# UBC-AWP/vision-sam3-yolo-lameless

Measured on AMD Instinct MI355X. Metric: frames/sec (whole node) for YOLO+SAM3+DINOv3 feature extraction, 1080p clips, higher is better.
Workload: dtype f16; 1 GPU; BASELINE cfg#5, dense schedule: fused per-frame path on a synthetic 5 s @ 30 fps 1080p clip (150 unique BGR frames resident in HBM): YOLOv8-l detect (letterbox 384x640, NMS, scale_boxes; f16 plan) -> SAM (Hiera-B+ image encoder + FPN at 1024x1024, box-prompted mask decoder, 1080p mask + statistics + contour features) + DINOv3 ViT-L/16 embed (224x224) on EVERY frame; per-frame records packed, gathe; parallelism=one clip per GPU, 1 GPU(s), one gather per step, streams=7

## Files before the change

### vision-sam3-yolo-lameless_amd/csrc/common.h

```cpp
#pragma once
#include <hip/hip_runtime.h>
#include <stdint.h>
#include <stdio.h>
#include <stdarg.h>
#include "../../include/lmx.h"

typedef _Float16 half_t;
typedef _Float16 half2_t __attribute__((ext_vector_type(2)));
typedef _Float16 half4_t __attribute__((ext_vector_type(4)));
typedef _Float16 half8_t __attribute__((ext_vector_type(8)));
typedef float f32x4 __attribute__((ext_vector_type(4)));
typedef float f32x16 __attribute__((ext_vector_type(16)));
typedef unsigned int u32x4 __attribute__((ext_vector_type(4)));
typedef unsigned int u32x2 __attribute__((ext_vector_type(2)));

void lmx_set_error(const char* fmt, ...);

#define LMX_REQUIRE(cond, ...)            \
  do {                                    \
    if (!(cond)) {                        \
      lmx_set_error(__VA_ARGS__);         \
      return LMX_EINVAL;                  \
    }                                     \
  } while (0)
// ... 53 lines not shown
  p = p * u + -8.481037793e-09f;
  p = p * u + 2.798429583e-07f;
  p = p * u + -6.151207192e-06f;
  p = p * u + 9.615961466e-05f;
  p = p * u + -1.114801972e-03f;
  p = p * u + 9.814679350e-03f;
  p = p * u + -6.632144717e-02f;
  p = p * u + 3.988863025e-01f;
  const f32x2 g = vc * p;
  return v * g + 0.5f * v;
}
__device__ __forceinline__ float gelu_1(float v) {
  const f32x2 r = gelu_pk(f32x2{v, v});
  return r[0];
}

__device__ __forceinline__ float lmx_act(float v, int act) {
  if (act == LMX_ACT_SILU) return v * __builtin_amdgcn_rcpf(1.0f + __builtin_amdgcn_exp2f(-v * 1.44269504088896340736f));
  if (act == LMX_ACT_GELU) return gelu_1(v);
  if (act == LMX_ACT_RELU) return fmaxf(v, 0.0f);
  return v;
}

typedef __attribute__((address_space(3))) void* lds_ptr_t;

__device__ __forceinline__ void lds_dma16(__amdgpu_buffer_rsrc_t rs, char* dst_lds, unsigned voffset, int soffset) {
  __builtin_amdgcn_raw_ptr_buffer_load_lds(rs, (lds_ptr_t)dst_lds, 16, voffset, soffset, 0, 0);
}

#define LMX_WAIT_CASE(n) \
  if constexpr (N == n) asm volatile("s_waitcnt vmcnt(" #n ")" ::: "memory")
template <int N>
__device__ __forceinline__ void wait_vmcnt() {
  static_assert(N == 0 || N == 1 || N == 2 || N == 3 || N == 4 || N == 6 || N == 8 || N == 9 || N == 12 || N == 16 || N == 18 || N == 24 ||
                    N == 32,
                "add the literal for this count");
  LMX_WAIT_CASE(0);
  LMX_WAIT_CASE(1);
  LMX_WAIT_CASE(2);
  LMX_WAIT_CASE(3);
  LMX_WAIT_CASE(4);
  LMX_WAIT_CASE(6);
  LMX_WAIT_CASE(8);
  LMX_WAIT_CASE(9);
  LMX_WAIT_CASE(12);
  LMX_WAIT_CASE(16);
  LMX_WAIT_CASE(18);
  LMX_WAIT_CASE(24);
  LMX_WAIT_CASE(32);
}
#undef LMX_WAIT_CASE
template <int PT>
__device__ __forceinline__ void wait_tiles(int y) {
  if (y >= 4)
    wait_vmcnt<4 * PT>();
  else if (y == 3)
    wait_vmcnt<3 * PT>();
  else if (y == 2)
    wait_vmcnt<2 * PT>();
  else if (y == 1)
    wait_vmcnt<PT>();
  else
    wait_vmcnt<0>();
}

static inline bool aligned16(const void* p) { return (((uintptr_t)p) & 15) == 0; }

__device__ __forceinline__ float wave_sum(float v) {
#pragma unroll
  for (int o = 32; o > 0; o >>= 1) v += __shfl_xor(v, o, 64);
  return v;
}
__device__ __forceinline__ float wave_max(float v) {
#pragma unroll
  for (int o = 32; o > 0; o >>= 1) v = fmaxf(v, __shfl_xor(v, o, 64));
  return v;
}

__device__ __forceinline__ float act_exact(float v, int act) {
  if (act == LMX_ACT_SILU) return v / (1.0f + expf(-v));
  if (act == LMX_ACT_RELU) return fmaxf(v, 0.0f);
  if (act == LMX_ACT_GELU) return 0.5f * v * (1.0f + erff(v * 0.70710678118654752440f));
// ... 21 lines not shown
```

### vision-sam3-yolo-lameless_amd/csrc/gemm2.hip

```cpp
#include "common.h"
#include <stdlib.h>
#include <type_traits>

#ifdef LMX_DBG_TIMELINE
__device__ unsigned long long lmx_tl[8 * 16384];
extern "C" int lmx_dbg_get_timeline(void* host, int64_t bytes) { return (int)hipMemcpyFromSymbol(host, HIP_SYMBOL(lmx_tl), bytes); }
#define TL(i, v) if (threadIdx.x == 0 && swz < 16384) lmx_tl[swz * 8 + (i)] = (v)
#else
#define TL(i, v)
#endif
namespace lmx_gemm2 {

__device__ __forceinline__ float act_apply(float v, int act) { return lmx_act(v, act); }

constexpr int smem_bytes(int BM, int BN, int BK, int NSTAGE) { return NSTAGE * (BM + BN) * BK * 2 + 2 * BN * 4; }
constexpr int waves_per_simd(int BM, int BN, int BK, int NSTAGE) {
  const int smem = smem_bytes(BM, BN, BK, NSTAGE), nwave = (BM / 64) * (BN / 64);
  const int wps = (smem <= 80 * 1024 ? 2 : 1) * nwave / 4;
  return wps < 1 ? 1 : wps;
}
template <int OUT_DT, int BM, int BN, int BK, int NSTAGE, int AMODE, int STAG, bool GATED = false>
__global__ __launch_bounds__(waves_per_simd(BM, BN, BK, NSTAGE) * 256) void gemm2_kernel(const lmx_gemm_desc p, const int ntiles, const int nt_ok) {
  constexpr int NWAVE = (BM / 64) * (BN / 64);
  constexpr int STAGE_BYTES = (BM + BN) * BK * 2;
  constexpr int A_INSTR = BM * BK * 2 / 1024 / NWAVE;
  constexpr int W_INSTR = BN * BK * 2 / 1024 / NWAVE;
  constexpr int ROWS_PER_INSTR = 1024 / (BK * 2);
  constexpr int CHUNKS = BK / 8;
  constexpr int LA = NSTAGE - 1;
  extern __shared__ __attribute__((aligned(16))) char smem[];
  const int tid = threadIdx.x;
  const int lane = tid & 63;
  const int wave = __builtin_amdgcn_readfirstlane(tid >> 6);
  const int wm = wave % (BM / 64), wn = wave / (BM / 64);

  const int bid = blockIdx.x, xcd = bid & 7;
  const int q = ntiles >> 3, r = ntiles & 7;
  const int base = xcd < r ? xcd * (q + 1) : r * (q + 1) + (xcd - r) * q;
  const int cnt = q + (xcd < r ? 1 : 0);
  const int stride = ((int)gridDim.x + 7 - xcd) >> 3;
  const int NT = (p.N + BN - 1) / BN;
  for (int li = bid >> 3; li < cnt; li += stride) {
  const int swz = base + li;
  const int S_ = p.split_k > 1 ? p.split_k : 1;
  const int tile_ = swz / S_, sp_ = swz - tile_ * S_;
  const int mt = tile_ / NT, nt = tile_ - mt * NT;
  const int m0 = mt * BM, n0 = nt * BN;
  TL(0, (unsigned long long)__builtin_amdgcn_s_getreg((31 << 11) | 4));
  TL(1, (unsigned long long)__builtin_amdgcn_s_getreg((31 << 11) | 20));
  TL(2, wall_clock64());
  TL(5, (unsigned long long)bid);

  const int hw_out = (AMODE == 1) ? p.Ho * p.Wo : 1;
  const int img0 = (AMODE == 1) ? m0 / hw_out : 0;
  const char* Ab = reinterpret_cast<const char*>(p.A) +
                   ((AMODE == 1) ? (int64_t)img0 * p.H * p.W_ * p.lda * 2 : (AMODE == 2 ? (int64_t)0 : (int64_t)m0 * p.lda * 2));
// ... 55 lines not shown
      const int kta = kt - (kt >= nkA ? nkA : 0) - (kt >= 2 * nkA ? nkA : 0);
      const int soff_a = (AMODE == 0) ? kta * (BK * 2) : soff;
#pragma unroll
      for (int j = 0; j < A_INSTR; ++j) {
        char* dst = st + (wave * A_INSTR + j) * 1024;
        lds_dma16(a_rs, dst, kill ? OOB : a_off[j], soff_a);
      }
    } else {
      const int k0 = kt * BK;
      const int tap = k0 / p.Cin, ci0 = k0 - tap * p.Cin;
      const int ky = tap / 3, kx = tap - 3 * ky;
      const int tap_off = ((ky * p.W_ + kx) * (int)p.lda + ci0) * 2;
#pragma unroll
      for (int j = 0; j < A_INSTR; ++j) {
        char* dst = st + (wave * A_INSTR + j) * 1024;
        const int iy = (a_yx[j] >> 16) + ky, ix = (int)(short)(a_yx[j] & 0xffff) + kx;
        const bool ok = (unsigned)iy < (unsigned)p.H && (unsigned)ix < (unsigned)p.W_;
        lds_dma16(a_rs, dst, ok ? a_off[j] + (unsigned)tap_off : OOB, 0);
      }
    }
#pragma unroll
    for (int j = 0; j < W_INSTR; ++j) {
      char* dst = st + BM * BK * 2 + (wave * W_INSTR + j) * 1024;
      lds_dma16(w_rs, dst, kill ? OOB : w_off[j], soff);
    }
  };

  f32x4 acc[4][4];
#pragma unroll
  for (int i = 0; i < 4; ++i)
#pragma unroll
    for (int j = 0; j < 4; ++j) acc[i][j] = f32x4{0.f, 0.f, 0.f, 0.f};

  float* bl = reinterpret_cast<float*>(smem + NSTAGE * STAGE_BYTES);
  float bias_v = 0.f, scale_v = 1.f;
  if (AMODE != 1 && tid < BN && n0 + tid < p.N) {
    if (p.bias && sp_ == 0) bias_v = p.bias[n0 + tid];
    if constexpr (GATED) {
      if (p.scale && tid < BN / 2 && (n0 >> 1) + tid < (p.N >> 1)) scale_v = p.scale[(n0 >> 1) + tid];
    } else {
      if (p.scale) scale_v = p.scale[n0 + tid];
    }
  }

#pragma unroll
  for (int t = 0; t < LA; ++t)
    if (t < nloc) issue(kt0 + t, t);

  const int frow = lane & 15, fq = lane >> 4;
  const int fsw = (BK == 64) ? (frow & 7) : ((-(frow >> 2)) & 3);
  constexpr int PT = A_INSTR + W_INSTR;
  if constexpr (STAG == 0) {
  for (int kt = 0; kt < nloc; ++kt) {
    const int left = nloc - 1 - kt;
    wait_tiles<PT>(left < LA - 1 ? left : LA - 1);
    __builtin_amdgcn_s_barrier();
#ifdef LMX_DBG_TIMELINE
    if (kt == 0) { TL(6, wall_clock64()); }
    if (kt == 1) { TL(7, wall_clock64()); }
#endif
    if (kt + LA < nloc) issue(kt0 + kt + LA, (kt + LA) % NSTAGE);
    const char* st = smem + (kt % NSTAGE) * STAGE_BYTES;
    const half_t* as = reinterpret_cast<const half_t*>(st) + (wm * 64 + frow) * BK;
    const half_t* ws = reinterpret_cast<const half_t*>(st + BM * BK * 2) + (wn * 64 + frow) * BK;
#ifdef LMX_DBG_NOMFMA
    if (p.M < 0)
#endif
// ... 30 lines not shown
#pragma unroll
    for (int ks = 0; ks < BK / 32; ++ks) {
      const int coff = (((ks << 2) + fq) ^ fsw) << 3;
#pragma unroll
      for (int j = 0; j < 4; ++j) wf[ks][j] = *reinterpret_cast<const half8_t*>(ws + j * 16 * BK + coff);
#pragma unroll
      for (int i = 0; i < 4; ++i) af[ks][i] = *reinterpret_cast<const half8_t*>(as + i * 16 * BK + coff);
    }
    if (kt + 1 < nloc) {
      const int rest = nloc - 2 - kt;
      wait_tiles<PT>(rest < LA - 2 ? (rest < 0 ? 0 : rest) : (LA - 2 < 0 ? 0 : LA - 2));
    }
    if (kt + LA < nloc) issue(kt0 + kt + LA, (kt + LA) % NSTAGE);
    asm volatile("s_waitcnt lgkmcnt(0)" ::: "memory");
    __builtin_amdgcn_s_barrier();
    __builtin_amdgcn_s_setprio(1);
#pragma unroll
    for (int ks = 0; ks < BK / 32; ++ks)
#pragma unroll
      for (int i = 0; i < 4; ++i)
#pragma unroll
        for (int j = 0; j < 4; ++j)
          acc[i][j] = __builtin_amdgcn_mfma_f32_16x16x32_f16(wf[ks][j], af[ks][i], acc[i][j], 0, 0, 0);
    __builtin_amdgcn_s_setprio(0);
    __builtin_amdgcn_s_barrier();
  }
  if (!grp) __builtin_amdgcn_s_barrier();
  }

  if (AMODE == 1 && tid < BN && n0 + tid < p.N) {
    if (p.bias && sp_ == 0) bias_v = p.bias[n0 + tid];
    if (p.scale) scale_v = p.scale[n0 + tid];
  }
  if (tid < BN) {
    bl[tid] = bias_v;
    bl[BN + tid] = scale_v;
  }
  asm volatile("s_waitcnt lgkmcnt(0)" ::: "memory");
  __builtin_amdgcn_s_barrier();
  TL(3, wall_clock64());
#ifdef LMX_DBG_NOEPI
  if (p.M > 0 && acc[0][0][0] != 12345.f) continue;
#endif
  const bool nt_out = nt_ok && OUT_DT == LMX_F16 && ((p.ldc * 2) & 127) == 0 && (int64_t)p.M * p.N >= (16ll << 20);
  char* my = smem + wave * 4608;
  auto epilogue = [&](auto act_c, auto scale_c) {
    constexpr int ACT = decltype(act_c)::value;
    constexpr bool SCALE = decltype(scale_c)::value;
    const float* blj = bl + wn * 64 + fq * 4;
    auto finish = [&](f32x4 v, int j) -> f32x4 {
      v += *reinterpret_cast<const f32x4*>(blj + j * 16);
      if constexpr (ACT == LMX_ACT_GELU) {
        const f32x2 g0 = gelu_pk(f32x2{v[0], v[1]}), g1 = gelu_pk(f32x2{v[2], v[3]});
        v = f32x4{g0[0], g0[1], g1[0], g1[1]};
      } else if constexpr (ACT != LMX_ACT_NONE) {
#pragma unroll
        for (int e = 0; e < 4; ++e) v[e] = act_apply(v[e], ACT);
      }
      if constexpr (SCALE) v *= *reinterpret_cast<const f32x4*>(blj + BN + j * 16);
      return v;
    };
    if constexpr (ACT == LMX_ACT_SWIGLU) {
      if constexpr (OUT_DT == LMX_F16 && AMODE == 0) {
        half_t* t16 = reinterpret_cast<half_t*>(my);
        constexpr int RS = 40;
        const bool nt_g = nt_ok && ((p.ldc * 2) & 127) == 0 && (int64_t)p.M * p.N >= (32ll << 20);
// ... 132 lines not shown
          const int m = m0 + wm * 64 + pass * 16 + row;
          if (m < p.M && n < p.N) {
            if (has_res) o += rr[it];
            *reinterpret_cast<f32x4*>(Cs + (int64_t)m * p.ldc + n) = o;
          }
        }
      }
    }
  };
  {
    using T = std::true_type;
    using F = std::false_type;
    const int act = p.act;
    if constexpr (GATED) {
      if (p.scale) epilogue(std::integral_constant<int, LMX_ACT_SWIGLU>{}, T{});
      else epilogue(std::integral_constant<int, LMX_ACT_SWIGLU>{}, F{});
    } else if (p.scale) {
      if (act == LMX_ACT_NONE) epilogue(std::integral_constant<int, LMX_ACT_NONE>{}, T{});
      else if (act == LMX_ACT_SILU) epilogue(std::integral_constant<int, LMX_ACT_SILU>{}, T{});
      else if (act == LMX_ACT_GELU) epilogue(std::integral_constant<int, LMX_ACT_GELU>{}, T{});
      else epilogue(std::integral_constant<int, LMX_ACT_RELU>{}, T{});
    } else {
      if (act == LMX_ACT_NONE) epilogue(std::integral_constant<int, LMX_ACT_NONE>{}, F{});
      else if (act == LMX_ACT_SILU) epilogue(std::integral_constant<int, LMX_ACT_SILU>{}, F{});
      else if (act == LMX_ACT_GELU) epilogue(std::integral_constant<int, LMX_ACT_GELU>{}, F{});
      else epilogue(std::integral_constant<int, LMX_ACT_RELU>{}, F{});
    }
  }
  __builtin_amdgcn_s_barrier();
  TL(4, wall_clock64());
  }
}

template <int BM, int BN, int BK, int NSTAGE, int AMODE, int STAG = 0>
int launch2(const lmx_gemm_desc& d, hipStream_t st) {
  const int MT = (d.M + BM - 1) / BM, NT = (d.N + BN - 1) / BN;
  const size_t smem = smem_bytes(BM, BN, BK, NSTAGE);
  int dev;
  LMX_TRY(lmx_stream_device(st, &dev));
  LMX_TRY(lmx_allow_lds(reinterpret_cast<const void*>(&gemm2_kernel<LMX_F16, BM, BN, BK, NSTAGE, AMODE, STAG>), (int)smem, dev));
  LMX_TRY(lmx_allow_lds(reinterpret_cast<const void*>(&gemm2_kernel<LMX_F32, BM, BN, BK, NSTAGE, AMODE, STAG>), (int)smem, dev));
  const int ntiles = MT * NT * (d.split_k > 1 ? d.split_k : 1);
  int grid = ntiles;
  static const int persist = lmx_env_int("LMX_GEMM2_PERSIST", 0);
  static const int nt_ok = !lmx_env_set("LMX_GEMM2_NO_NT");
  if (persist > 0 && grid > 256 * persist) grid = 256 * persist;
  if (d.act == LMX_ACT_SWIGLU) {
    if constexpr (AMODE == 0) {
      LMX_TRY(lmx_allow_lds(reinterpret_cast<const void*>(&gemm2_kernel<LMX_F16, BM, BN, BK, NSTAGE, AMODE, STAG, true>), (int)smem, dev));
      hipLaunchKernelGGL((gemm2_kernel<LMX_F16, BM, BN, BK, NSTAGE, AMODE, STAG, true>), dim3(grid), dim3(BM * BN / 64), smem, st, d, ntiles, nt_ok);
      return lmx_launch_check("gemm2_kernel (gated)");
    } else {
      return LMX_EINVAL;
    }
  }
  if (d.out_dtype == LMX_F16)
    hipLaunchKernelGGL((gemm2_kernel<LMX_F16, BM, BN, BK, NSTAGE, AMODE, STAG>), dim3(grid), dim3(BM * BN / 64), smem, st, d, ntiles, nt_ok);
  else
    hipLaunchKernelGGL((gemm2_kernel<LMX_F32, BM, BN, BK, NSTAGE, AMODE, STAG>), dim3(grid), dim3(BM * BN / 64), smem, st, d, ntiles, nt_ok);
  return lmx_launch_check("gemm2_kernel");
}

constexpr int RL_BM = 128, RL_BN = 448, RL_BK = 64, RL_NSTAGE = 2;
constexpr int RL_STAGE_BYTES = (RL_BM + RL_BN) * RL_BK * 2;
constexpr int RL_RS = RL_BN + 4;
constexpr int RL_SMEM = RL_NSTAGE * RL_STAGE_BYTES + 3 * RL_BN * 4;
static_assert(2 * 32 * RL_RS * 4 <= RL_NSTAGE * RL_STAGE_BYTES, "two 32-row epilogue buffers inside the ring");

__device__ __forceinline__ void wave_sum4(float (&v)[4]) {
#pragma unroll
  for (int o = 32; o > 0; o >>= 1) {
    float t[4];
#pragma unroll
    for (int r = 0; r < 4; ++r) t[r] = __shfl_xor(v[r], o, 64);
#pragma unroll
    for (int r = 0; r < 4; ++r) v[r] += t[r];
  }
}

__global__ __launch_bounds__(512) void gemm2_rowln_kernel(const lmx_gemm_desc p) {
  constexpr int BM = RL_BM, BN = RL_BN, BK = RL_BK, NSTAGE = RL_NSTAGE, STAGE_BYTES = RL_STAGE_BYTES;
  constexpr int NWAVE = 8;
  constexpr int A_INSTR = BM * BK * 2 / 1024 / NWAVE;
  constexpr int W_INSTR = BN * BK * 2 / 1024 / NWAVE;
  constexpr int FJ = BN / 4 / 16;
  extern __shared__ __attribute__((aligned(16))) char smem[];
  const int tid = threadIdx.x;
  const int lane = tid & 63;
  const int wave = __builtin_amdgcn_readfirstlane(tid >> 6);
  const int wm = wave & 1, wn = wave >> 1;
  const int swz = blockIdx.x;
  const int m0 = swz * BM;
// ... 151 lines not shown
          *reinterpret_cast<half4_t*>(Lh + (int64_t)m * p.ld_ln + c0) = half4_t{(half_t)o[0], (half_t)o[1], (half_t)o[2], (half_t)o[3]};
        }
        if (ok1) {
          const f32x4 o = (v1[rr] - mean[rr]) * rstd[rr] * g1 + b1;
          *reinterpret_cast<half4_t*>(Lh + (int64_t)m * p.ld_ln + c1) = half4_t{(half_t)o[0], (half_t)o[1], (half_t)o[2], (half_t)o[3]};
        }
      }
    }
  }
  TL(4, wall_clock64());
}

int launch_rowln(const lmx_gemm_desc& d, hipStream_t st) {
  int dev;
  LMX_TRY(lmx_stream_device(st, &dev));
  LMX_TRY(lmx_allow_lds(reinterpret_cast<const void*>(&gemm2_rowln_kernel), RL_SMEM, dev));
  hipLaunchKernelGGL(gemm2_rowln_kernel, dim3((d.M + RL_BM - 1) / RL_BM), dim3(512), RL_SMEM, st, d);
  return lmx_launch_check("gemm2_rowln_kernel");
}

}
using namespace lmx_gemm2;

static int g_variant = -1;
extern "C" void lmx_dbg_set_gemm2_variant(int v) { g_variant = v; }

static constexpr GemmRoute tiling(int BM, int BN, int BK, int NSTAGE, int STAG = 0) { return GemmRoute{true, BM, BN, BK, NSTAGE, STAG}; }

GemmRoute lmx_gemm2_tiling(const lmx_gemm_desc& d) {
  if (g_variant < 0) g_variant = lmx_env_char("LMX_GEMM2_VARIANT");
  if (d.a_mode == 2) return tiling(256, 256, 64, 2);
  if (d.a_mode == 1) {
    static const int conv_small = lmx_env_set("LMX_GEMM2_CONV_SMALL");
    const int64_t t256 = (int64_t)((d.M + 255) / 256) * ((d.N + 255) / 256);
    const double q256 = (double)t256 / (double)(((t256 + 255) / 256) * 256);
    if (!conv_small && d.N % 256 == 0 && t256 >= 230 && q256 >= 0.75) return tiling(256, 256, 32, 3, 1);
    return tiling(256, 128, 32, 3);
  }
  switch (g_variant) {
    case 'A': return tiling(256, 128, 64, 3);
    case 'B': return tiling(128, 128, 64, 2);
    case 'C': return tiling(256, 128, 32, 3);
    case 'D': return tiling(256, 128, 32, 2);
    case 'E': return tiling(256, 256, 32, 3);
    case 'F': return tiling(256, 256, 32, 4);
    case 'H': return tiling(128, 128, 32, 2);
    case 'I': return tiling(128, 128, 32, 3);
    case 'S': return tiling(256, 128, 32, 6, 1);
    case 'T': return tiling(256, 128, 64, 3, 1);
    case 'U': return tiling(256, 128, 32, 3, 1);
    case 'V': return tiling(256, 128, 32, 4, 1);
    case 'W': return tiling(256, 256, 32, 4, 1);
    case 'Y': return tiling(256, 256, 32, 3, 1);
    case 'Z': return tiling(256, 256, 64, 2);
  }
  const int64_t nt256 = (d.N + 255) / 256, tiles256 = (int64_t)((d.M + 255) / 256) * nt256;
  const double nfrac = (double)d.N / (double)(nt256 * 256);
  const double q256 = (double)tiles256 / (double)(((tiles256 + 255) / 256) * 256);
  if (d.K >= 448 && tiles256 >= 200 && q256 >= 0.75 && nfrac >= 0.85) {
    return tiling(256, 256, 64, 2);
  }
  if (d.K < 448 && d.N >= 224 && d.N <= 1536 && d.N % 256 != 0 && nfrac >= 0.85 && tiles256 >= 200 && q256 >= 0.75)
    return d.K > 128 ? tiling(256, 256, 32, 3) : tiling(256, 256, 64, 2);
  const int64_t tiles = (int64_t)((d.M + 255) / 256) * ((d.N + 127) / 128);
  return (d.K >= 1792 || tiles <= 256) ? tiling(256, 128, 64, 3, 1) : tiling(256, 128, 32, 3);
}

static constexpr int64_t tiling_key(int BM, int BN, int BK, int NSTAGE, int a_mode, int STAG) {
  return ((((int64_t)BM * 1024 + BN) * 1024 + BK) * 16 + NSTAGE) * 16 + a_mode * 2 + STAG;
}

int lmx_gemm2_launch(const lmx_gemm_desc& d, const GemmRoute& r, hipStream_t st) {
  if (r.rowln) return launch_rowln(d, st);
#define LMX_T(BM, BN, BK, NSTAGE, AMODE, STAG) \
  case tiling_key(BM, BN, BK, NSTAGE, AMODE, STAG): return launch2<BM, BN, BK, NSTAGE, AMODE, STAG>(d, st)
  switch (tiling_key(r.BM, r.BN, r.BK, r.NSTAGE, d.a_mode, r.STAG)) {
    LMX_T(256, 256, 64, 2, 2, 0);
    LMX_T(256, 256, 32, 3, 1, 1);
    LMX_T(256, 128, 32, 3, 1, 0);
    LMX_T(256, 128, 64, 3, 0, 0);
    LMX_T(128, 128, 64, 2, 0, 0);
    LMX_T(256, 128, 32, 3, 0, 0);
    LMX_T(256, 128, 32, 2, 0, 0);
    LMX_T(256, 256, 32, 3, 0, 0);
    LMX_T(256, 256, 32, 4, 0, 0);
    LMX_T(128, 128, 32, 2, 0, 0);
    LMX_T(128, 128, 32, 3, 0, 0);
    LMX_T(256, 128, 32, 6, 0, 1);
    LMX_T(256, 128, 64, 3, 0, 1);
    LMX_T(256, 128, 32, 3, 0, 1);
    LMX_T(256, 128, 32, 4, 0, 1);
    LMX_T(256, 256, 32, 4, 0, 1);
    LMX_T(256, 256, 32, 3, 0, 1);
    LMX_T(256, 256, 64, 2, 0, 0);
  }
#undef LMX_T
  LMX_REQUIRE(false, "lmx_k_gemm: no LDS-DMA kernel %dx%dx%d, %d slots, staggered %d for a_mode %d", r.BM, r.BN, r.BK, r.NSTAGE, r.STAG, d.a_mode);
}
```

### vision-sam3-yolo-lameless_amd/csrc/yolo.hip

```cpp
#include "common.h"

namespace {

inline int grid_for(int64_t total, int block = 256) {
  int64_t g = (total + block - 1) / block;
  if (g > 256 * 8) g = 256 * 8;
  if (g < 1) g = 1;
  return (int)g;
}

__global__ __launch_bounds__(256) void letterbox_kernel(const uint8_t* __restrict__ src, uint8_t* __restrict__ dst, int n,
                                                        int sh, int sw, int rh, int rw, int top, int left, int oh, int ow,
                                                        const int* __restrict__ xofs, const short* __restrict__ ialpha,
                                                        const int* __restrict__ yofs, const short* __restrict__ ibeta,
                                                        int swap_rb, int identity) {
  const int64_t total = (int64_t)n * oh * ow;
  for (int64_t i = (int64_t)blockIdx.x * blockDim.x + threadIdx.x; i < total; i += (int64_t)gridDim.x * blockDim.x) {
    const int ox = (int)(i % ow);
    const int64_t r = i / ow;
    const int oy = (int)(r % oh);
    const int img = (int)(r / oh);
    uint8_t* d = dst + i * 3;
    const int dy = oy - top, dx = ox - left;
    if (dy < 0 || dy >= rh || dx < 0 || dx >= rw) {
// ... 7 lines not shown
      v[0] = s[0];
      v[1] = s[1];
      v[2] = s[2];
    } else {
      const int sx0 = xofs[dx];
      const int sx1 = sx0 + 1 < sw ? sx0 + 1 : sw - 1;
      const int a0 = ialpha[2 * dx], a1 = ialpha[2 * dx + 1];
      int sy0 = yofs[dy], sy1 = yofs[dy] + 1;
      sy0 = sy0 < 0 ? 0 : (sy0 < sh ? sy0 : sh - 1);
      sy1 = sy1 < 0 ? 0 : (sy1 < sh ? sy1 : sh - 1);
      const int b0 = ibeta[2 * dy], b1 = ibeta[2 * dy + 1];
      const uint8_t* r0 = S + (int64_t)sy0 * sw * 3;
      const uint8_t* r1 = S + (int64_t)sy1 * sw * 3;
#pragma unroll
      for (int c = 0; c < 3; ++c) {
        const int h0 = (int)r0[sx0 * 3 + c] * a0 + (int)r0[sx1 * 3 + c] * a1;
        const int h1 = (int)r1[sx0 * 3 + c] * a0 + (int)r1[sx1 * 3 + c] * a1;
        const int val = (((b0 * (h0 >> 4)) >> 16) + ((b1 * (h1 >> 4)) >> 16) + 2) >> 2;
        v[c] = (uint8_t)(val < 0 ? 0 : (val > 255 ? 255 : val));
      }
    }
    if (swap_rb) {
      d[0] = v[2];
      d[1] = v[1];
      d[2] = v[0];
    } else {
      d[0] = v[0];
      d[1] = v[1];
      d[2] = v[2];
    }
  }
}

template <int CO_T>
__global__ __launch_bounds__(256) void stem_conv_kernel(const uint8_t* __restrict__ img, const float* __restrict__ w,
                                                        const float* __restrict__ bias, half_t* __restrict__ out, int n,
                                                        int H, int W, int Ho, int Wo, int Cout) {
  extern __shared__ __attribute__((aligned(16))) char smem[];
  float* ws = reinterpret_cast<float*>(smem);
  for (int i = threadIdx.x; i < 27 * Cout; i += blockDim.x) ws[i] = w[i];
  for (int i = threadIdx.x; i < Cout; i += blockDim.x) ws[27 * Cout + i] = bias[i];
  __syncthreads();
  const int64_t total = (int64_t)n * Ho * Wo;
  for (int64_t i = (int64_t)blockIdx.x * blockDim.x + threadIdx.x; i < total; i += (int64_t)gridDim.x * blockDim.x) {
    const int ox = (int)(i % Wo);
    const int64_t r = i / Wo;
    const int oy = (int)(r % Ho);
    const int b = (int)(r / Ho);
    float x[27];
#pragma unroll
    for (int ky = 0; ky < 3; ++ky)
#pragma unroll
      for (int kx = 0; kx < 3; ++kx) {
        const int iy = oy * 2 - 1 + ky, ix = ox * 2 - 1 + kx;
        const bool ok = (unsigned)iy < (unsigned)H && (unsigned)ix < (unsigned)W;
        const uint8_t* s = img + (((int64_t)b * H + (ok ? iy : 0)) * W + (ok ? ix : 0)) * 3;
#pragma unroll
        for (int c = 0; c < 3; ++c) x[(ky * 3 + kx) * 3 + c] = ok ? (float)s[c] / 255.0f : 0.0f;
      }
    half_t* o = out + i * Cout;
    for (int c0 = 0; c0 < Cout; c0 += CO_T) {
      float acc[CO_T];
#pragma unroll
      for (int j = 0; j < CO_T; ++j) acc[j] = ws[27 * Cout + c0 + j];
#pragma unroll
      for (int t = 0; t < 27; ++t) {
        const float xv = x[t];
#pragma unroll
        for (int j = 0; j < CO_T; ++j) acc[j] = fmaf(xv, ws[t * Cout + c0 + j], acc[j]);
      }
      half8_t hv;
#pragma unroll
      for (int j = 0; j < CO_T; ++j) {
        const float v = acc[j] / (1.0f + expf(-acc[j]));
        hv[j] = (half_t)v;
      }
      *reinterpret_cast<half8_t*>(o + c0) = hv;
    }
  }
}

__global__ __launch_bounds__(256) void maxpool5_kernel(const half_t* __restrict__ src, int64_t lds, half_t* __restrict__ dst,
                                                       int64_t ldd, int n, int H, int W, int C) {
  const int cc = C / 8;
  const int64_t total = (int64_t)n * H * W * cc;
  for (int64_t i = (int64_t)blockIdx.x * blockDim.x + threadIdx.x; i < total; i += (int64_t)gridDim.x * blockDim.x) {
    const int c = (int)(i % cc) * 8;
    const int64_t p = i / cc;
    const int x = (int)(p % W);
    const int64_t r = p / W;
    const int y = (int)(r % H);
    const int b = (int)(r / H);
    half8_t m;
#pragma unroll
    for (int e = 0; e < 8; ++e) m[e] = (half_t)(-65504.0f);
    for (int dy = -2; dy <= 2; ++dy) {
      const int yy = y + dy;
      if ((unsigned)yy >= (unsigned)H) continue;
      for (int dx = -2; dx <= 2; ++dx) {
        const int xx = x + dx;
        if ((unsigned)xx >= (unsigned)W) continue;
        const half8_t v = *reinterpret_cast<const half8_t*>(src + (((int64_t)b * H + yy) * W + xx) * lds + c);
#pragma unroll
        for (int e = 0; e < 8; ++e) m[e] = v[e] > m[e] ? v[e] : m[e];
      }
    }
    *reinterpret_cast<half8_t*>(dst + p * ldd + c) = m;
  }
}

__global__ __launch_bounds__(256) void upsample2_kernel(const half_t* __restrict__ src, int64_t lds, half_t* __restrict__ dst,
// ... 142 lines not shown
  for (int l = 0; l < 3; ++l) {
    LMX_REQUIRE(hw[2 * l] > 0 && hw[2 * l + 1] > 0, "lmx_k_pose_gather: level %d geometry", l);
    L.h[l] = hw[2 * l];
    L.w[l] = hw[2 * l + 1];
    L.off[l] = off;
    L.stride[l] = strides[l];
    off += L.h[l] * L.w[l];
  }
  hipLaunchKernelGGL(pose_gather_kernel, dim3(grid_for((int64_t)n * max_det * K)), dim3(256), 0,
                     reinterpret_cast<hipStream_t>(stream), L, ldk, src, counts, n, max_det, K, ndim, padx, pady, gain, w, h, out);
  return lmx_launch_check("pose_gather_kernel");
}

extern "C" int lmx_k_letterbox(const uint8_t* src, uint8_t* dst, int n, int sh, int sw, int rh, int rw, int top, int left,
                               int oh, int ow, const int32_t* xofs, const int16_t* ialpha, const int32_t* yofs,
                               const int16_t* ibeta, int swap_rb, lmx_stream_t stream) {
  LMX_REQUIRE(src && dst, "lmx_k_letterbox: null pointer");
  LMX_REQUIRE(n > 0 && sh > 0 && sw > 0 && rh > 0 && rw > 0 && oh >= top + rh && ow >= left + rw && top >= 0 && left >= 0,
              "lmx_k_letterbox: geometry");
  const int identity = (rh == sh && rw == sw) ? 1 : 0;
  LMX_REQUIRE(identity || (xofs && ialpha && yofs && ibeta), "lmx_k_letterbox: null tables");
  hipLaunchKernelGGL(letterbox_kernel, dim3(grid_for((int64_t)n * oh * ow)), dim3(256), 0,
                     reinterpret_cast<hipStream_t>(stream), src, dst, n, sh, sw, rh, rw, top, left, oh, ow, xofs, ialpha, yofs,
                     ibeta, swap_rb, identity);
  return lmx_launch_check("letterbox_kernel");
}

extern "C" int lmx_k_stem_conv(const uint8_t* img, const float* w, const float* bias, void* out, int n, int H, int W, int Cout,
                               lmx_stream_t stream) {
  LMX_REQUIRE(img && w && bias && out, "lmx_k_stem_conv: null pointer");
  LMX_REQUIRE(n > 0 && H > 0 && W > 0 && Cout > 0 && Cout % 8 == 0 && Cout <= 256, "lmx_k_stem_conv: shape (Cout %d)", Cout);
  LMX_REQUIRE(aligned16(out), "lmx_k_stem_conv: out alignment");
  const int Ho = (H + 2 - 3) / 2 + 1, Wo = (W + 2 - 3) / 2 + 1;
  const size_t smem = (size_t)28 * Cout * sizeof(float);
  hipLaunchKernelGGL((stem_conv_kernel<8>), dim3(grid_for((int64_t)n * Ho * Wo)), dim3(256), smem,
                     reinterpret_cast<hipStream_t>(stream), img, w, bias, reinterpret_cast<half_t*>(out), n, H, W, Ho, Wo, Cout);
  return lmx_launch_check("stem_conv_kernel");
}

extern "C" int lmx_k_maxpool5(const void* src, int64_t lds, void* dst, int64_t ldd, int n, int H, int W, int C,
                              lmx_stream_t stream) {
  LMX_REQUIRE(src && dst, "lmx_k_maxpool5: null pointer");
  LMX_REQUIRE(n > 0 && H > 0 && W > 0 && C > 0 && C % 8 == 0 && lds % 8 == 0 && ldd % 8 == 0 && lds >= C && ldd >= C,
              "lmx_k_maxpool5: shape");
  LMX_REQUIRE(aligned16(src) && aligned16(dst), "lmx_k_maxpool5: alignment");
  hipLaunchKernelGGL(maxpool5_kernel, dim3(grid_for((int64_t)n * H * W * (C / 8))), dim3(256), 0,
                     reinterpret_cast<hipStream_t>(stream), reinterpret_cast<const half_t*>(src), lds,
                     reinterpret_cast<half_t*>(dst), ldd, n, H, W, C);
  return lmx_launch_check("maxpool5_kernel");
}

extern "C" int lmx_k_upsample2(const void* src, int64_t lds, void* dst, int64_t ldd, int n, int H, int W, int C,
                               lmx_stream_t stream) {
  LMX_REQUIRE(src && dst, "lmx_k_upsample2: null pointer");
  LMX_REQUIRE(n > 0 && H > 0 && W > 0 && C > 0 && C % 8 == 0 && lds % 8 == 0 && ldd % 8 == 0 && lds >= C && ldd >= C,
              "lmx_k_upsample2: shape");
  LMX_REQUIRE(aligned16(src) && aligned16(dst), "lmx_k_upsample2: alignment");
  hipLaunchKernelGGL(upsample2_kernel, dim3(grid_for((int64_t)n * 4 * H * W * (C / 8))), dim3(256), 0,
                     reinterpret_cast<hipStream_t>(stream), reinterpret_cast<const half_t*>(src), lds,
                     reinterpret_cast<half_t*>(dst), ldd, n, H, W, C);
  return lmx_launch_check("upsample2_kernel");
}

extern "C" int lmx_k_detect_decode(const float* head, int64_t ldh, float* pred, int n, int H, int W, int nc, float stride,
                                   int a_off, int A, lmx_stream_t stream) {
  LMX_REQUIRE(head && pred, "lmx_k_detect_decode: null pointer");
  LMX_REQUIRE(n > 0 && H > 0 && W > 0 && nc > 0 && a_off >= 0 && a_off + H * W <= A, "lmx_k_detect_decode: shape");
  LMX_REQUIRE(ldh >= 64 + nc && ldh % 4 == 0 && aligned16(head), "lmx_k_detect_decode: head row stride %lld", (long long)ldh);
  hipLaunchKernelGGL(detect_decode_kernel, dim3(grid_for((int64_t)n * H * W * 4)), dim3(256), 0,
// ... 12 lines not shown
```

Measured before the change: 802.0 frames/s.

## Rewrite YOLO stem conv with register weights and add deeper conv GEMM tilings

The YOLO stem conv is restructured so that each thread keeps the weights for a group of 4 output channels in registers. The input patches are staged through double-buffered LDS using a u8-to-float lookup table, and the next chunk's gather is prefetched while the current one is computed. Two new f16-only implicit-GEMM conv tilings (256x256x64 and 256x64x64, 2 stages) are selected for large-K or 64-channel convolutions. Those tilings place the bias/scale scratch inside the ring so occupancy stays at two waves per SIMD. This adds an extra barrier, more vmcnt literals and register pressure in the stem.

```diff
diff --git a/vision-sam3-yolo-lameless_amd/csrc/common.h b/vision-sam3-yolo-lameless_amd/csrc/common.h
--- a/vision-sam3-yolo-lameless_amd/csrc/common.h
+++ b/vision-sam3-yolo-lameless_amd/csrc/common.h
@@ -109,8 +109,8 @@
   if constexpr (N == n) asm volatile("s_waitcnt vmcnt(" #n ")" ::: "memory")
 template <int N>
 __device__ __forceinline__ void wait_vmcnt() {
-  static_assert(N == 0 || N == 1 || N == 2 || N == 3 || N == 4 || N == 6 || N == 8 || N == 9 || N == 12 || N == 16 || N == 18 || N == 24 ||
-                    N == 32,
+  static_assert(N == 0 || N == 1 || N == 2 || N == 3 || N == 4 || N == 6 || N == 8 || N == 9 || N == 10 || N == 12 ||
+                    N == 16 || N == 18 || N == 20 || N == 24 || N == 30 || N == 32 || N == 40,
                 "add the literal for this count");
   LMX_WAIT_CASE(0);
   LMX_WAIT_CASE(1);
@@ -120,11 +120,15 @@
   LMX_WAIT_CASE(6);
   LMX_WAIT_CASE(8);
   LMX_WAIT_CASE(9);
+  LMX_WAIT_CASE(10);
   LMX_WAIT_CASE(12);
   LMX_WAIT_CASE(16);
   LMX_WAIT_CASE(18);
+  LMX_WAIT_CASE(20);
   LMX_WAIT_CASE(24);
+  LMX_WAIT_CASE(30);
   LMX_WAIT_CASE(32);
+  LMX_WAIT_CASE(40);
 }
 #undef LMX_WAIT_CASE
 template <int PT>
diff --git a/vision-sam3-yolo-lameless_amd/csrc/gemm2.hip b/vision-sam3-yolo-lameless_amd/csrc/gemm2.hip
--- a/vision-sam3-yolo-lameless_amd/csrc/gemm2.hip
+++ b/vision-sam3-yolo-lameless_amd/csrc/gemm2.hip
@@ -13,15 +13,24 @@
 
 __device__ __forceinline__ float act_apply(float v, int act) { return lmx_act(v, act); }
 
-constexpr int smem_bytes(int BM, int BN, int BK, int NSTAGE) { return NSTAGE * (BM + BN) * BK * 2 + 2 * BN * 4; }
-constexpr int waves_per_simd(int BM, int BN, int BK, int NSTAGE) {
-  const int smem = smem_bytes(BM, BN, BK, NSTAGE), nwave = (BM / 64) * (BN / 64);
+constexpr bool bl_in_ring(int BM, int BN, int BK, int NSTAGE, int AMODE) {
+  const int ring = NSTAGE * (BM + BN) * BK * 2;
+  return AMODE == 1 && ring <= 80 * 1024 && ring + 2 * BN * 4 > 80 * 1024;
+}
+constexpr int smem_bytes(int BM, int BN, int BK, int NSTAGE, int AMODE = 0) {
+  return NSTAGE * (BM + BN) * BK * 2 + (bl_in_ring(BM, BN, BK, NSTAGE, AMODE) ? 0 : 2 * BN * 4);
+}
+constexpr int waves_per_simd(int BM, int BN, int BK, int NSTAGE, int AMODE = 0) {
+  const int smem = smem_bytes(BM, BN, BK, NSTAGE, AMODE), nwave = (BM / 64) * (BN / 64);
   const int wps = (smem <= 80 * 1024 ? 2 : 1) * nwave / 4;
   return wps < 1 ? 1 : wps;
 }
 template <int OUT_DT, int BM, int BN, int BK, int NSTAGE, int AMODE, int STAG, bool GATED = false>
-__global__ __launch_bounds__(waves_per_simd(BM, BN, BK, NSTAGE) * 256) void gemm2_kernel(const lmx_gemm_desc p, const int ntiles, const int nt_ok) {
+__global__ __launch_bounds__(waves_per_simd(BM, BN, BK, NSTAGE, AMODE) * 256) void gemm2_kernel(const lmx_gemm_desc p, const int ntiles, const int nt_ok) {
   constexpr int NWAVE = (BM / 64) * (BN / 64);
+  constexpr bool BL_IN_RING = bl_in_ring(BM, BN, BK, NSTAGE, AMODE);
+  static_assert(BM * BK * 2 / 1024 >= NWAVE && BN * BK * 2 / 1024 >= NWAVE, "every wave issues at least one LDS-DMA of A and of W per k-tile");
+  static_assert(NWAVE * 4608 <= NSTAGE * (BM + BN) * BK * 2 - (BL_IN_RING ? 2 * BN * 4 : 0), "the epilogue's per-wave slices lie inside the ring");
   constexpr int STAGE_BYTES = (BM + BN) * BK * 2;
   constexpr int A_INSTR = BM * BK * 2 / 1024 / NWAVE;
   constexpr int W_INSTR = BN * BK * 2 / 1024 / NWAVE;
@@ -143,7 +152,7 @@
 #pragma unroll
     for (int j = 0; j < 4; ++j) acc[i][j] = f32x4{0.f, 0.f, 0.f, 0.f};
 
-  float* bl = reinterpret_cast<float*>(smem + NSTAGE * STAGE_BYTES);
+  float* bl = reinterpret_cast<float*>(smem + NSTAGE * STAGE_BYTES - (BL_IN_RING ? 2 * BN * 4 : 0));
   float bias_v = 0.f, scale_v = 1.f;
   if (AMODE != 1 && tid < BN && n0 + tid < p.N) {
     if (p.bias && sp_ == 0) bias_v = p.bias[n0 + tid];
@@ -240,6 +249,10 @@
     if (p.bias && sp_ == 0) bias_v = p.bias[n0 + tid];
     if (p.scale) scale_v = p.scale[n0 + tid];
   }
+  if constexpr (BL_IN_RING) {
+    asm volatile("s_waitcnt lgkmcnt(0)" ::: "memory");
+    __builtin_amdgcn_s_barrier();
+  }
   if (tid < BN) {
     bl[tid] = bias_v;
     bl[BN + tid] = scale_v;
@@ -438,14 +451,15 @@
   }
 }
 
-template <int BM, int BN, int BK, int NSTAGE, int AMODE, int STAG = 0>
+template <int BM, int BN, int BK, int NSTAGE, int AMODE, int STAG = 0, bool F32_TOO = true>
 int launch2(const lmx_gemm_desc& d, hipStream_t st) {
   const int MT = (d.M + BM - 1) / BM, NT = (d.N + BN - 1) / BN;
-  const size_t smem = smem_bytes(BM, BN, BK, NSTAGE);
+  const size_t smem = smem_bytes(BM, BN, BK, NSTAGE, AMODE);
   int dev;
   LMX_TRY(lmx_stream_device(st, &dev));
   LMX_TRY(lmx_allow_lds(reinterpret_cast<const void*>(&gemm2_kernel<LMX_F16, BM, BN, BK, NSTAGE, AMODE, STAG>), (int)smem, dev));
-  LMX_TRY(lmx_allow_lds(reinterpret_cast<const void*>(&gemm2_kernel<LMX_F32, BM, BN, BK, NSTAGE, AMODE, STAG>), (int)smem, dev));
+  if constexpr (F32_TOO)
+    LMX_TRY(lmx_allow_lds(reinterpret_cast<const void*>(&gemm2_kernel<LMX_F32, BM, BN, BK, NSTAGE, AMODE, STAG>), (int)smem, dev));
   const int ntiles = MT * NT * (d.split_k > 1 ? d.split_k : 1);
   int grid = ntiles;
   static const int persist = lmx_env_int("LMX_GEMM2_PERSIST", 0);
@@ -460,10 +474,14 @@
       return LMX_EINVAL;
     }
   }
-  if (d.out_dtype == LMX_F16)
+  if (d.out_dtype == LMX_F16) {
     hipLaunchKernelGGL((gemm2_kernel<LMX_F16, BM, BN, BK, NSTAGE, AMODE, STAG>), dim3(grid), dim3(BM * BN / 64), smem, st, d, ntiles, nt_ok);
-  else
-    hipLaunchKernelGGL((gemm2_kernel<LMX_F32, BM, BN, BK, NSTAGE, AMODE, STAG>), dim3(grid), dim3(BM * BN / 64), smem, st, d, ntiles, nt_ok);
+  } else {
+    if constexpr (F32_TOO)
+      hipLaunchKernelGGL((gemm2_kernel<LMX_F32, BM, BN, BK, NSTAGE, AMODE, STAG>), dim3(grid), dim3(BM * BN / 64), smem, st, d, ntiles, nt_ok);
+    else
+      LMX_REQUIRE(false, "lmx_k_gemm: the %dx%dx%d tiling is built for f16 output only", BM, BN, BK);
+  }
   return lmx_launch_check("gemm2_kernel");
 }
 
@@ -681,9 +699,12 @@
   if (d.a_mode == 2) return tiling(256, 256, 64, 2);
   if (d.a_mode == 1) {
     static const int conv_small = lmx_env_set("LMX_GEMM2_CONV_SMALL");
+    const bool deep = d.out_dtype == LMX_F16 && d.split_k <= 1 && d.Cin % 64 == 0;
     const int64_t t256 = (int64_t)((d.M + 255) / 256) * ((d.N + 255) / 256);
     const double q256 = (double)t256 / (double)(((t256 + 255) / 256) * 256);
-    if (!conv_small && d.N % 256 == 0 && t256 >= 230 && q256 >= 0.75) return tiling(256, 256, 32, 3, 1);
+    if (!conv_small && d.N % 256 == 0 && t256 >= 230 && q256 >= 0.75)
+      return deep && d.K >= 2304 ? tiling(256, 256, 64, 2) : tiling(256, 256, 32, 3, 1);
+    if (deep && d.N == 64 && d.Cin == 64 && d.M >= 65536) return tiling(256, 64, 64, 2);
     return tiling(256, 128, 32, 3);
   }
   switch (g_variant) {
@@ -723,10 +744,14 @@
   if (r.rowln) return launch_rowln(d, st);
 #define LMX_T(BM, BN, BK, NSTAGE, AMODE, STAG) \
   case tiling_key(BM, BN, BK, NSTAGE, AMODE, STAG): return launch2<BM, BN, BK, NSTAGE, AMODE, STAG>(d, st)
+#define LMX_T16(BM, BN, BK, NSTAGE, AMODE, STAG) \
+  case tiling_key(BM, BN, BK, NSTAGE, AMODE, STAG): return launch2<BM, BN, BK, NSTAGE, AMODE, STAG, false>(d, st)
   switch (tiling_key(r.BM, r.BN, r.BK, r.NSTAGE, d.a_mode, r.STAG)) {
     LMX_T(256, 256, 64, 2, 2, 0);
     LMX_T(256, 256, 32, 3, 1, 1);
     LMX_T(256, 128, 32, 3, 1, 0);
+    LMX_T16(256, 64, 64, 2, 1, 0);
+    LMX_T16(256, 256, 64, 2, 1, 0);
     LMX_T(256, 128, 64, 3, 0, 0);
     LMX_T(128, 128, 64, 2, 0, 0);
     LMX_T(256, 128, 32, 3, 0, 0);
@@ -744,5 +769,6 @@
     LMX_T(256, 256, 64, 2, 0, 0);
   }
 #undef LMX_T
+#undef LMX_T16
   LMX_REQUIRE(false, "lmx_k_gemm: no LDS-DMA kernel %dx%dx%d, %d slots, staggered %d for a_mode %d", r.BM, r.BN, r.BK, r.NSTAGE, r.STAG, d.a_mode);
 }
diff --git a/vision-sam3-yolo-lameless_amd/csrc/yolo.hip b/vision-sam3-yolo-lameless_amd/csrc/yolo.hip
--- a/vision-sam3-yolo-lameless_amd/csrc/yolo.hip
+++ b/vision-sam3-yolo-lameless_amd/csrc/yolo.hip
@@ -63,51 +63,108 @@
   }
 }
 
-template <int CO_T>
+constexpr int STEM_CO = 4;
+constexpr int STEM_XS = 28;
+inline int stem_pixb(int Cout) { return 256 / (Cout / STEM_CO); }
+inline int stem_passes(int Cout) { const int pb = stem_pixb(Cout); return pb >= 128 ? 1 : 128 / pb; }
 __global__ __launch_bounds__(256) void stem_conv_kernel(const uint8_t* __restrict__ img, const float* __restrict__ w,
                                                         const float* __restrict__ bias, half_t* __restrict__ out, int n,
-                                                        int H, int W, int Ho, int Wo, int Cout) {
+                                                        int H, int W, int Ho, int Wo, int Cout, int PIXB, int passes, int64_t nchunks) {
   extern __shared__ __attribute__((aligned(16))) char smem[];
-  float* ws = reinterpret_cast<float*>(smem);
-  for (int i = threadIdx.x; i < 27 * Cout; i += blockDim.x) ws[i] = w[i];
-  for (int i = threadIdx.x; i < Cout; i += blockDim.x) ws[27 * Cout + i] = bias[i];
+  float* lut = reinterpret_cast<float*>(smem);
+  float* xs = lut + 256;
+  const int tid = threadIdx.x;
+  const int G = Cout / STEM_CO, CP = PIXB * passes;
+  const bool worker = tid < PIXB * G;
+  const int g = tid % G, lp0 = tid / G;
+  const int64_t total = (int64_t)n * Ho * Wo;
+  lut[tid] = (float)tid / 255.0f;
+
+  f32x2 wr[27][STEM_CO / 2], br[STEM_CO / 2];
+#pragma unroll
+  for (int h = 0; h < STEM_CO / 2; ++h) br[h] = f32x2{bias[g * STEM_CO + 2 * h], bias[g * STEM_CO + 2 * h + 1]};
+#pragma unroll
+  for (int t = 0; t < 27; ++t)
+#pragma unroll
+    for (int h = 0; h < STEM_CO / 2; ++h) wr[t][h] = f32x2{w[t * Cout + g * STEM_CO + 2 * h], w[t * Cout + g * STEM_CO + 2 * h + 1]};
+
+  int v[27];
+  unsigned inside = 0;
+  auto request = [&](int64_t P0) {
+    const int64_t gp = P0 + tid;
+    if (tid < CP && gp < total) {
+      const int ox = (int)(gp % Wo);
+      const int64_t r = gp / Wo;
+      const int oy = (int)(r % Ho);
+      const int64_t b = r / Ho;
+      inside = 0;
+#pragma unroll
+      for (int ky = 0; ky < 3; ++ky)
+#pragma unroll
+        for (int kx = 0; kx < 3; ++kx) {
+          const int iy = oy * 2 - 1 + ky, ix = ox * 2 - 1 + kx;
+          const bool ok = (unsigned)iy < (unsigned)H && (unsigned)ix < (unsigned)W;
+          const uint8_t* s = img + ((b * H + (ok ? iy : 0)) * W + (ok ? ix : 0)) * 3;
+          inside |= (ok ? 1u : 0u) << (ky * 3 + kx);
+#pragma unroll
+          for (int c = 0; c < 3; ++c) v[(ky * 3 + kx) * 3 + c] = s[c];
+        }
+    }
+  };
+  auto stage = [&](int64_t P0, float* dst) {
+    if (tid < CP && P0 + tid < total) {
+      float* d = dst + tid * STEM_XS;
+#pragma unroll
+      for (int t = 0; t < 27; ++t) {
+        const float f = lut[v[t]];
+        d[t] = ((inside >> (t / 3)) & 1) ? f : 0.0f;
+      }
+      d[27] = 0.0f;
+    }
+  };
+
+  int64_t c = blockIdx.x;
+  request(c * CP);
   __syncthreads();
-  const int64_t total = (int64_t)n * Ho * Wo;
-  for (int64_t i = (int64_t)blockIdx.x * blockDim.x + threadIdx.x; i < total; i += (int64_t)gridDim.x * blockDim.x) {
-    const int ox = (int)(i % Wo);
-    const int64_t r = i / Wo;
-    const int oy = (int)(r % Ho);
-    const int b = (int)(r / Ho);
-    float x[27];
-#pragma unroll
-    for (int ky = 0; ky < 3; ++ky)
-#pragma unroll
-      for (int kx = 0; kx < 3; ++kx) {
-        const int iy = oy * 2 - 1 + ky, ix = ox * 2 - 1 + kx;
-        const bool ok = (unsigned)iy < (unsigned)H && (unsigned)ix < (unsigned)W;
-        const uint8_t* s = img + (((int64_t)b * H + (ok ? iy : 0)) * W + (ok ? ix : 0)) * 3;
-#pragma unroll
-        for (int c = 0; c < 3; ++c) x[(ky * 3 + kx) * 3 + c] = ok ? (float)s[c] / 255.0f : 0.0f;
-      }
-    half_t* o = out + i * Cout;
-    for (int c0 = 0; c0 < Cout; c0 += CO_T) {
-      float acc[CO_T];
-#pragma unroll
-      for (int j = 0; j < CO_T; ++j) acc[j] = ws[27 * Cout + c0 + j];
-#pragma unroll
-      for (int t = 0; t < 27; ++t) {
-        const float xv = x[t];
-#pragma unroll
-        for (int j = 0; j < CO_T; ++j) acc[j] = fmaf(xv, ws[t * Cout + c0 + j], acc[j]);
-      }
-      half8_t hv;
-#pragma unroll
-      for (int j = 0; j < CO_T; ++j) {
-        const float v = acc[j] / (1.0f + expf(-acc[j]));
-        hv[j] = (half_t)v;
-      }
-      *reinterpret_cast<half8_t*>(o + c0) = hv;
-    }
+  stage(c * CP, xs);
+  __syncthreads();
+  for (int it = 0; c < nchunks; c += gridDim.x, ++it) {
+    const int64_t P0 = c * CP, Pn = (c + gridDim.x) * CP;
+    const float* cur = xs + (it & 1) * CP * STEM_XS;
+    if (c + gridDim.x < nchunks) request(Pn);
+    if (worker) {
+      for (int ps = 0; ps < passes; ++ps) {
+        const int lp = lp0 + ps * PIXB;
+        const int64_t gp = P0 + lp;
+        if (gp >= total) break;
+        float x[STEM_XS];
+#pragma unroll
+        for (int q = 0; q < STEM_XS / 4; ++q) {
+          const f32x4 xv = *reinterpret_cast<const f32x4*>(cur + lp * STEM_XS + q * 4);
+          x[q * 4 + 0] = xv[0];
+          x[q * 4 + 1] = xv[1];
+          x[q * 4 + 2] = xv[2];
+          x[q * 4 + 3] = xv[3];
+        }
+        f32x2 acc[STEM_CO / 2];
+#pragma unroll
+        for (int h = 0; h < STEM_CO / 2; ++h) acc[h] = br[h];
+#pragma unroll
+        for (int t = 0; t < 27; ++t)
+#pragma unroll
+          for (int h = 0; h < STEM_CO / 2; ++h) acc[h] = __builtin_elementwise_fma(f32x2{x[t], x[t]}, wr[t][h], acc[h]);
+        half4_t hv;
+#pragma unroll
+        for (int j = 0; j < STEM_CO; ++j) {
+          const float a = acc[j >> 1][j & 1];
+          const float s = a / (1.0f + expf(-a));
+          hv[j] = (half_t)s;
+        }
+        *reinterpret_cast<half4_t*>(out + gp * Cout + g * STEM_CO) = hv;
+      }
+    }
+    if (c + gridDim.x < nchunks) stage(Pn, xs + ((it + 1) & 1) * CP * STEM_XS);
+    __syncthreads();
   }
 }
 
@@ -316,9 +373,11 @@
   LMX_REQUIRE(n > 0 && H > 0 && W > 0 && Cout > 0 && Cout % 8 == 0 && Cout <= 256, "lmx_k_stem_conv: shape (Cout %d)", Cout);
   LMX_REQUIRE(aligned16(out), "lmx_k_stem_conv: out alignment");
   const int Ho = (H + 2 - 3) / 2 + 1, Wo = (W + 2 - 3) / 2 + 1;
-  const size_t smem = (size_t)28 * Cout * sizeof(float);
-  hipLaunchKernelGGL((stem_conv_kernel<8>), dim3(grid_for((int64_t)n * Ho * Wo)), dim3(256), smem,
-                     reinterpret_cast<hipStream_t>(stream), img, w, bias, reinterpret_cast<half_t*>(out), n, H, W, Ho, Wo, Cout);
+  const int PIXB = stem_pixb(Cout), passes = stem_passes(Cout), CP = PIXB * passes;
+  const int64_t nchunks = ((int64_t)n * Ho * Wo + CP - 1) / CP;
+  const size_t smem = (size_t)(256 + 2 * CP * STEM_XS) * sizeof(float);
+  hipLaunchKernelGGL(stem_conv_kernel, dim3(grid_for(nchunks, 1)), dim3(256), smem, reinterpret_cast<hipStream_t>(stream), img, w,
+                     bias, reinterpret_cast<half_t*>(out), n, H, W, Ho, Wo, Cout, PIXB, passes, nchunks);
   return lmx_launch_check("stem_conv_kernel");
 }
 
```

Result: no change. 807.8 frames/s, median of 6 (+0.7%).
